# baurst/rbrt

Measured on NVIDIA B200. Metric: Mrays/s, higher is better.
Workload: dtype f32

## Files before the change

rbrt_b200/csrc/api.cu:

```cuda
#include <dlfcn.h>
#include <chrono>
#include <cstdarg>
#include <cstdio>
#include <cstring>
#include "aov.cuh"
#include "bvh_build.cuh"
#include "engine.cuh"
#include "multi.cuh"
#include "query.cuh"
#include "update.cuh"

namespace rbrt {

static thread_local char g_err[512] = "";
void set_error(const char* fmt, ...) {
    va_list ap; va_start(ap, fmt); vsnprintf(g_err, sizeof(g_err), fmt, ap); va_end(ap);
}
int cuda_fail(cudaError_t e, const char* what) {
    set_error("CUDA error %d (%s) at %s", (int)e, cudaGetErrorString(e), what);
    cudaGetLastError();
    return (e == cudaErrorNoDevice || e == cudaErrorInsufficientDriver) ? RBRT_E_NODEVICE : RBRT_E_CUDA;
}
std::recursive_mutex& api_mutex() { static std::recursive_mutex m; return m; }
static uint64_t g_pool_limit = 0;
uint64_t pool_limit_bytes() { return g_pool_limit; }

static int g_device = -1;
static double now_ms() {
    return std::chrono::duration<double, std::milli>(std::chrono::steady_clock::now().time_since_epoch()).count();
}

#define CKA(x) do { cudaError_t e_ = (x); if (e_ != cudaSuccess) return cuda_fail(e_, #x); } while (0)
#define LOCK std::lock_guard<std::recursive_mutex> lock_(api_mutex())

int current_device() { return g_device; }
void set_current_device(int d) { g_device = d; }

static int ensure_device() {
    if (g_device >= 0) { CKA(cudaSetDevice(g_device)); return RBRT_OK; }
    int n = 0;
    cudaError_t e = cudaGetDeviceCount(&n);
    if (e != cudaSuccess || n == 0) {
        set_error("no CUDA device available (%s); rbrt_b200 has no CPU fallback", e != cudaSuccess ? cudaGetErrorString(e) : "device count 0");
        cudaGetLastError();
        return RBRT_E_NODEVICE;
    }
    g_device = 0;
    CKA(cudaSetDevice(0));
    return RBRT_OK;
}

int device_sm_count(int device, int* out) {
    static int cached[64] = {0};
    if (!cached[device & 63]) {
        int smc = 0;
        cudaError_t e = cudaDeviceGetAttribute(&smc, cudaDevAttrMultiProcessorCount, device);
        if (e != cudaSuccess) return cuda_fail(e, "cudaDeviceGetAttribute");
        cached[device & 63] = smc;
    }
    *out = cached[device & 63];
    return RBRT_OK;
// ... 232 lines not shown
        float4* d_tris = (float4*)(base + sc->lay.tris) + 3ull * md.tri_base;
        float4* d_normals = (float4*)(base + sc->lay.nrm) + md.nrm_base;
        float4* d_nodes = (float4*)(base + sc->lay.nodes) + 4ull * md.node_base;
        BuildResult* d_res = (BuildResult*)(base + sc->lay.result) + mi;
        if (mat) {
            Scene::Staging* sg = nullptr;
            { int rc = stage_get(sc, 32, &sg); if (rc) return rc; }
            const float4 m4 = make_float4(mat->albedo.x, mat->albedo.y, mat->albedo.z, mat->param);
            memcpy(sg->p, &m4, 16); memcpy((char*)sg->p + 16, &mat->kind, 4);
            const size_t e = sc->n_elems + mi;
            CKA(cudaMemcpyAsync(base + sc->lay.mat + 16 * e, sg->p, 16, cudaMemcpyHostToDevice, ctx.build));
            CKA(cudaMemcpyAsync(base + sc->lay.kind + 4 * e, (char*)sg->p + 16, 4, cudaMemcpyHostToDevice, ctx.build));
            CKA(cudaEventRecord(sg->done, ctx.build));
        }
        if (flags == RBRT_UPDATE_REBUILD) {
            CKA(build_mesh(ctx, verts, n, n_eff, sc->pad_rel, sc->leaf_size, sc->sah, md, d_mesh, d_tris, d_normals, d_nodes, d_res,
                           on_device ? sc->upd_in : nullptr));
            if (!on_device) {
                { int rc = ensure_event(&sc->t_up1); if (rc) return rc; }
                CKA(build_uploads_done(ctx, sc->t_up1)); uploaded = sc->t_up1;
            }
            { int rc = ensure_event(&sc->rebuild_ev); if (rc) return rc; }
            CKA(cudaMemcpyAsync((BuildResult*)sc->res_h + mi, d_res, sizeof(BuildResult), cudaMemcpyDeviceToHost, ctx.build));
            CKA(cudaEventRecord(sc->rebuild_ev, ctx.build));
            sc->rebuild_pending = true;
        } else {
            const size_t raw_bytes = on_device ? 0 : (36ull * n + 255) & ~255ull;
            char* sbase = nullptr;
            CKA(build_slot_acquire(ctx, raw_bytes + um->scratch_bytes(n_eff), &sbase));
            if (!on_device && n) CKA(cudaMemcpyAsync(sbase, verts, 36ull * n, cudaMemcpyHostToDevice, ctx.copy));
            CKA(build_slot_uploaded(ctx, &uploaded));
            if (on_device) CKA(cudaStreamWaitEvent(ctx.build, sc->upd_in, 0));
            RefitArgs a;
            a.raw = on_device ? verts : (const float*)sbase; a.n_all = n; a.n_eff = n_eff; a.pad_rel = sc->pad_rel;
            a.mesh = d_mesh; a.tris = d_tris; a.normals = d_normals; a.nodes = reinterpret_cast<uint4*>(d_nodes); a.res = d_res;
            CKA((cudaError_t)um->refit(&a, sbase + raw_bytes, ctx.build));
            CKA(build_slot_release(ctx));
            if (on_device) uploaded = nullptr;
        }
    }
    { int rc = update_end(sc, ctx); if (rc) return rc; }
    if (on_device && !receiver) {
        { int rc = ensure_event(&sc->upd_out); if (rc) return rc; }
        CKA(cudaEventRecord(sc->upd_out, ctx.build));
        CKA(cudaStreamWaitEvent(user_st, sc->upd_out, 0));
    }
    if (uploaded) CKA(cudaEventSynchronize(uploaded));
    return RBRT_OK;
}

struct LaunchModule { const char* env; const char* file; const char* what; const char* symbol; void* launch; };
static LaunchModule g_aov_module = {"RBRT_GPU_AOV_LIB", "librbrt_gpu_aov.so", "AOV", "rbrt_aov_launch", nullptr};
static LaunchModule g_query_module = {"RBRT_GPU_QUERY_LIB", "librbrt_gpu_query.so", "query", "rbrt_query_launch", nullptr};
static int load_module(LaunchModule& m) {
    if (!m.launch) {
        std::string path;
        { int rc = module_path(m.env, m.file, &path); if (rc) return rc; }
        void* h = dlopen(path.c_str(), RTLD_NOW | RTLD_LOCAL);
        if (!h) { set_error("the %s module is missing (dlopen %s: %s); build it with make -C rbrt_b200/csrc", m.what, path.c_str(), dlerror()); return RBRT_E_CUDA; }
        void* f = dlsym(h, m.symbol);
        if (!f) { set_error("%s lacks the %s entry point", path.c_str(), m.what); dlclose(h); return RBRT_E_CUDA; }
        m.launch = f;
    }
    return RBRT_OK;
}

struct AovPool { char* buf = nullptr; size_t bytes = 0; unsigned long long* ctr = nullptr; cudaEvent_t e0 = nullptr, e1 = nullptr; };
static AovPool g_aov[64];
static void aov_release_all() {
    int cur = 0; cudaGetDevice(&cur);
    for (int d = 0; d < 64; ++d) {
        AovPool& p = g_aov[d];
        if (!p.buf && !p.ctr && !p.e0) continue;
        cudaSetDevice(d);
        cudaFree(p.buf); cudaFree(p.ctr);
        if (p.e0) cudaEventDestroy(p.e0);
        if (p.e1) cudaEventDestroy(p.e1);
        p = AovPool();
    }
    cudaSetDevice(cur);
}

static int render_aov(const rbrt_scene* scene, const rbrt_camera* cam, uint32_t spp, uint64_t seed, const rbrt_aov_out* out, bool host,
                      cudaStream_t st, rbrt_stats* stats) {
    if (!scene || !cam || !out) { set_error("null argument"); return RBRT_E_INVALID; }
    if (!out->depth && !out->normal && !out->albedo && !out->coverage && !out->hit_kind && !out->elem_idx && !out->tri_idx) {
        set_error("no AOV requested (every member of the output is NULL)"); return RBRT_E_INVALID;
    }
    const uint64_t n = (uint64_t)cam->img_width_pix * cam->img_height_pix;
    if (!n || !spp) { set_error("empty image or zero samples"); return RBRT_E_INVALID; }
    if (n > 0xFFFFFFFFull) { set_error("more than 2^32 - 1 pixels"); return RBRT_E_INVALID; }
    const Scene& sc = *reinterpret_cast<const Scene*>(scene);
    const Replica& rp = sc.rep[0];
    CKA(cudaSetDevice(rp.device));
    const double t0 = now_ms();
    if (stats) memset(stats, 0, sizeof(*stats));
    { int rc = resolve_scene_info(sc, true); if (rc) return rc; }
    { int rc = load_module(g_aov_module); if (rc) return rc; }
    const rbrt_aov_launch_fn launch = reinterpret_cast<rbrt_aov_launch_fn>(g_aov_module.launch);

    AovPool& pool = g_aov[rp.device & 63];
    AovArgs a;
    memset(&a, 0, sizeof(a));
    a.S = rp.dev; a.cam = make_cam(*cam); a.key0 = (uint32_t)seed; a.key1 = (uint32_t)(seed >> 32); a.n_samples = spp;
    a.tiles_x = (cam->img_width_pix + 7) / 8; a.tiles_total = a.tiles_x * ((cam->img_height_pix + 3) / 4);
    a.out = *out;
    if (host) {
        const size_t b1 = a256(4 * n), b3 = a256(12 * n);
        const size_t need = (out->depth ? b1 : 0) + (out->normal ? b3 : 0) + (out->albedo ? b3 : 0) + (out->coverage ? b1 : 0) +
                            (out->hit_kind ? b1 : 0) + (out->elem_idx ? b1 : 0) + (out->tri_idx ? b1 : 0);
        if (pool.bytes < need) {
            cudaFree(pool.buf); pool.buf = nullptr; pool.bytes = 0;
            CKA(cudaMalloc(&pool.buf, need)); pool.bytes = need;
        }
        char* p = pool.buf;
        auto take = [&](const void* want, size_t b) -> char* { if (!want) return nullptr; char* q = p; p += b; return q; };
// ... 609 lines not shown
```

rbrt_b200/csrc/engine.cuh:

```cuda
#pragma once
#include <mutex>
#include <string>
#include <vector>
#include "../../include/rbrt_gpu.h"
#include "common.cuh"

namespace rbrt {

struct IterCtr {
    uint32_t ray_count;
    uint32_t cand_count;
    uint32_t cand_head;
    uint32_t mat_count[3];
    uint32_t shade_head;
    uint32_t pad;
};

enum { ST_RAYS = 0, ST_NAN = 1, ST_NODES = 2, ST_TRIS = 3, ST_CAND = 4, ST_TAIL_NODES = 5, ST_TAIL_TRIS = 6, ST_TAIL_CAND = 7, ST_COUNT = 8 };

struct WaveBuffers {
    uint32_t cap = 0;
    uint32_t depth_cap = 0;
    uint4* rec = nullptr;
    uint32_t* candq = nullptr;
    uint32_t* matq[2][3] = {{nullptr, nullptr, nullptr}, {nullptr, nullptr, nullptr}};
    float4* out = nullptr;
    uint16_t* hist = nullptr;
    IterCtr* ctr = nullptr;
    unsigned long long* stats = nullptr;
    float4* accum = nullptr;
    size_t accum_px = 0;
    uint8_t* rgb = nullptr; float* hdr = nullptr; size_t out_px = 0;
    std::vector<cudaEvent_t> ev;
    size_t bytes = 0;
};

struct ArenaLayout { size_t nodes = 0, tris = 0, nrm = 0, sph = 0, mat = 0, kind = 0, mesh = 0, etris = 0, ekind = 0, result = 0, total = 0; };
struct Replica { int device = 0; char* arena = nullptr; size_t arena_bytes = 0; SceneDev dev{}; int sm_count = 148;
                 cudaEvent_t ready = nullptr; };
struct SceneUse { int device; cudaStream_t stream; cudaEvent_t ev; };

struct Scene {
    int device = 0;
    SceneDev dev{};
    std::vector<MeshDev> meshes_h;
    std::vector<Replica> rep;
    ArenaLayout lay{};
    uint32_t n_elems = 0, n_meshes = 0, n_etris = 0;
    rbrt_scene_info info{};
    int sm_count = 148;
    bool collective = false;
    mutable std::vector<SceneUse> uses;
    void* res_h = nullptr;
    cudaEvent_t info_ev = nullptr, t_up0 = nullptr, t_up1 = nullptr, t_b0 = nullptr, t_b1 = nullptr;
    mutable bool info_resolved = false;
    mutable int build_error = 0;
    double ms_host_create = 0;
    std::vector<uint64_t> mesh_n_all;
    std::vector<uint32_t> elem_kind_h;
    float pad_rel = 0.0f;
    uint32_t leaf_size = 1;
    bool sah = true;
    bool replicated = false;
    cudaEvent_t upd_in = nullptr, upd_out = nullptr;
    cudaEvent_t rebuild_ev = nullptr;
    mutable bool rebuild_pending = false;
    struct Staging { void* p = nullptr; size_t bytes = 0; cudaEvent_t done = nullptr; };
    Staging stage[2];
    int stage_next = 0;
};
int resolve_scene_info(const Scene& sc, bool wait);
void wait_scene_ready(const Scene& sc, int li, cudaStream_t st);
void wait_scene_uses(const Scene& sc, int device, cudaStream_t st);

struct WaveParams {
    SceneDev S;
    CamDev cam[RBRT_MAX_FRAMES];
    ShardDev sh;
    uint32_t key0[RBRT_MAX_FRAMES], key1[RBRT_MAX_FRAMES];
    uint32_t n_frames;
    FastDiv fd_s_count;
// ... 48 lines not shown
```

rbrt_b200/csrc/render.cu:

```cuda
#include <cstdio>
#include <algorithm>
#include <cstdlib>
#include <cstring>
#include "engine.cuh"
#include "intersect.cuh"
#include "cull.cuh"
#include "shade.cuh"

namespace rbrt {

#define FULL_MASK 0xFFFFFFFFu
#define CLS_CAND 3
#define CLS_NONE 7
#define ROUNDS 4

__device__ __forceinline__ uint32_t warp_append(uint32_t* counter, bool pred) {
    uint32_t mask = __ballot_sync(FULL_MASK, pred);
    if (mask == 0) return 0;
    uint32_t lane = threadIdx.x & 31;
    uint32_t leader = __ffs(mask) - 1;
    uint32_t base = 0;
    if (lane == leader) base = atomicAdd(counter, __popc(mask));
    base = __shfl_sync(FULL_MASK, base, leader);
    return base + __popc(mask & ((1u << lane) - 1));
}

__device__ __forceinline__ uint32_t warp_grab(uint32_t* head, uint32_t count) {
    uint32_t base = 0;
    if ((threadIdx.x & 31) == 0) base = atomicAdd(head, count);
    return __shfl_sync(FULL_MASK, base, 0);
}

struct Deferred {
    uint32_t cls;
    uint32_t pid[ROUNDS];
    __device__ __forceinline__ void clear() { cls = 0; for (int r = 0; r < ROUNDS; ++r) { cls |= (uint32_t)CLS_NONE << (3 * r); pid[r] = 0; } }
    __device__ __forceinline__ void set(int r, uint32_t c, uint32_t p) { cls = (cls & ~(7u << (3 * r))) | (c << (3 * r)); pid[r] = p; }
};

__device__ __forceinline__ void flush(const WaveParams& P, uint32_t it, const Deferred& df) {
    IterCtr* c = P.ctr + it;
    const uint32_t lane = threadIdx.x & 31, lt = (1u << lane) - 1;
#pragma unroll
    for (uint32_t k = 0; k < 4; ++k) {
        uint32_t m[ROUNDS], total = 0;
#pragma unroll
        for (int r = 0; r < ROUNDS; ++r) { m[r] = __ballot_sync(FULL_MASK, ((df.cls >> (3 * r)) & 7u) == k); total += __popc(m[r]); }
        if (total == 0) continue;
        uint32_t base = 0;
        if (lane == 0) base = atomicAdd(k == CLS_CAND ? &c->cand_count : &c->mat_count[k], total);
        base = __shfl_sync(FULL_MASK, base, 0);
        uint32_t* q = k == CLS_CAND ? P.candq : P.matq[it & 1][k];
#pragma unroll
        for (int r = 0; r < ROUNDS; ++r) {
            if (m[r] & (1u << lane)) q[base + __popc(m[r] & lt)] = df.pid[r];
            base += __popc(m[r]);
        }
    }
}

// ... 690 lines not shown
            out.elem_idx = elem;
        } else {
            const uint32_t mi = elem - P.S.n_spheres;
            const float4 nn = __ldg(P.S.normals + P.S.meshes[mi].nrm_base + tri); nrm = mk3(nn.x, nn.y, nn.z);
            out.kind = RBRT_HIT_MESH; out.elem_idx = mi; out.tri_idx = tri;
        }
        out.t = t; out.dist = len3(o - p);
        out.point.x = p.x; out.point.y = p.y; out.point.z = p.z;
        out.normal.x = nrm.x; out.normal.y = nrm.y; out.normal.z = nrm.z;
    }
    hits[pid] = out;
}

CamDev make_cam(const rbrt_camera& c) {
    CamDev d;
    d.pos[0] = c.position.x; d.pos[1] = c.position.y; d.pos[2] = c.position.z;
    d.right[0] = c.right.x; d.right[1] = c.right.y; d.right[2] = c.right.z;
    d.up[0] = c.up.x; d.up[1] = c.up.y; d.up[2] = c.up.z;
    d.center[0] = c.img_center_point.x; d.center[1] = c.img_center_point.y; d.center[2] = c.img_center_point.z;
    d.mm_per_pix_hor = c.mm_per_pix_hor; d.mm_per_pix_vert = c.mm_per_pix_vert;
    d.width = c.img_width_pix; d.height = c.img_height_pix;
    return d;
}

static WaveBuffers g_wave[8][64];
WaveBuffers& device_wave_buffers(int device, int pool) { return g_wave[pool & 7][(device >= 0 && device < 64) ? device : 0]; }
struct SplitLane { cudaStream_t aux = nullptr; cudaEvent_t fork = nullptr, acc[2] = {nullptr, nullptr}, join = nullptr; };
static SplitLane g_lane[4][64];
static int ensure_lane(SplitLane& L) {
    if (L.aux) return RBRT_OK;
    cudaError_t e = cudaStreamCreateWithFlags(&L.aux, cudaStreamNonBlocking);
    for (cudaEvent_t* ev : {&L.fork, &L.acc[0], &L.acc[1], &L.join}) if (e == cudaSuccess) e = cudaEventCreateWithFlags(ev, cudaEventDisableTiming);
    if (e != cudaSuccess) return cuda_fail(e, "split lane");
    return RBRT_OK;
}
void release_device_wave_buffers() {
    int cur = 0; cudaGetDevice(&cur);
    for (int p = 0; p < 8; ++p)
        for (int d = 0; d < 64; ++d) if (g_wave[p][d].cap || g_wave[p][d].accum || g_wave[p][d].rgb) { cudaSetDevice(d); free_wave_buffers(g_wave[p][d]); }
    for (int p = 0; p < 4; ++p)
        for (int d = 0; d < 64; ++d) {
            SplitLane& L = g_lane[p][d];
            if (!L.aux) continue;
            cudaSetDevice(d); cudaStreamSynchronize(L.aux); cudaStreamDestroy(L.aux);
            for (cudaEvent_t ev : {L.fork, L.acc[0], L.acc[1], L.join}) if (ev) cudaEventDestroy(ev);
            L = SplitLane();
        }
    cudaSetDevice(cur);
}

void free_wave_buffers(WaveBuffers& wb) {
    cudaFree(wb.rec); cudaFree(wb.candq);
    for (int i = 0; i < 6; ++i) cudaFree(wb.matq[i / 3][i % 3]);
    cudaFree(wb.out); cudaFree(wb.hist); cudaFree(wb.ctr); cudaFree(wb.stats); cudaFree(wb.accum);
    cudaFree(wb.rgb); cudaFree(wb.hdr);
    for (cudaEvent_t e : wb.ev) cudaEventDestroy(e);
    wb = WaveBuffers();
}

#define CKR(x) do { cudaError_t e_ = (x); if (e_ != cudaSuccess) return cuda_fail(e_, #x); } while (0)

static int ensure_wave_buffers(WaveBuffers& wb, uint32_t cap, uint32_t depth) {
    if (wb.cap >= cap && wb.depth_cap >= depth && wb.stats) return RBRT_OK;
    float4* accum = wb.accum; size_t accum_px = wb.accum_px; uint8_t* rgb = wb.rgb; float* hdr = wb.hdr; size_t out_px = wb.out_px;
    std::vector<cudaEvent_t> ev; ev.swap(wb.ev);
    wb.accum = nullptr; wb.rgb = nullptr; wb.hdr = nullptr;
    free_wave_buffers(wb);
    wb.accum = accum; wb.accum_px = accum_px; wb.rgb = rgb; wb.hdr = hdr; wb.out_px = out_px; wb.ev.swap(ev);
    size_t b = 0;
    CKR(cudaMalloc(&wb.rec, 32ull * cap)); b += 32ull * cap;
    CKR(cudaMalloc(&wb.candq, 4ull * cap)); b += 4ull * cap;
    for (int i = 0; i < 6; ++i) { CKR(cudaMalloc(&wb.matq[i / 3][i % 3], 4ull * cap)); b += 4ull * cap; }
    CKR(cudaMalloc(&wb.out, 16ull * cap)); b += 16ull * cap;
    { const uint64_t rows = std::max<uint64_t>(depth, 1); CKR(cudaMalloc(&wb.hist, 2ull * cap * rows)); b += 2ull * cap * rows; }
    CKR(cudaMalloc(&wb.ctr, sizeof(IterCtr) * (depth + 2)));
    CKR(cudaMalloc(&wb.stats, 8 * ST_COUNT));
    wb.cap = cap; wb.depth_cap = depth; wb.bytes = b;
    return RBRT_OK;
}

void note_scene_use(const Scene& sc, int device, cudaStream_t st) {
    static std::mutex mu;
    std::lock_guard<std::mutex> g(mu);
    for (SceneUse& u : sc.uses)
        if (u.device == device && u.stream == st) { cudaEventRecord(u.ev, st); return; }
    SceneUse u{device, st, nullptr};
    if (cudaEventCreateWithFlags(&u.ev, cudaEventDisableTiming) != cudaSuccess) { cudaGetLastError(); return; }
    cudaEventRecord(u.ev, st);
    sc.uses.push_back(u);
}

int make_shard(const rbrt_render_opts& o, uint32_t W, uint32_t H, uint32_t spp, ShardDev* out) {
    ShardDev sh;
    sh.rank = 0; sh.count = 1; sh.s0 = 0; sh.s1 = spp;
    sh.tiles_x = (W + 7) / 8;
    sh.fd_tiles_x = make_fastdiv(sh.tiles_x);
    sh.tiles_total = sh.tiles_x * ((H + 3) / 4);
    if (o.shard_count > 1) {
        if (o.shard_rank >= o.shard_count) { set_error("shard_rank >= shard_count"); return RBRT_E_INVALID; }
        if (o.shard_mode == RBRT_SHARD_TILES) { sh.rank = o.shard_rank; sh.count = o.shard_count; }
        else if (o.shard_mode == RBRT_SHARD_SAMPLES) {
            sh.s0 = (uint32_t)((uint64_t)spp * o.shard_rank / o.shard_count);
            sh.s1 = (uint32_t)((uint64_t)spp * (o.shard_rank + 1) / o.shard_count);
        } else { set_error("shard_count > 1 needs shard_mode TILES or SAMPLES"); return RBRT_E_INVALID; }
    }
    sh.tiles_mine = sh.tiles_total > sh.rank ? (sh.tiles_total - sh.rank + sh.count - 1) / sh.count : 0;
    *out = sh;
    return RBRT_OK;
}

int render_accum(const Scene& sc, int li, const rbrt_camera* cams, const uint64_t* seeds, uint32_t n_frames, uint32_t spp,
                 const rbrt_render_opts* opts, float4* const* d_accum, cudaStream_t st, rbrt_stats* stats, RenderJob* job_out) {
    const Replica& rp = sc.rep[li];
    RenderJob local_job;
    RenderJob& job = job_out ? *job_out : local_job;
    if (!n_frames || n_frames > RBRT_MAX_FRAMES) { set_error("n_frames must be 1..%d", RBRT_MAX_FRAMES); return RBRT_E_INVALID; }
    const rbrt_camera& cam = cams[0];
    const uint32_t W = cam.img_width_pix, H = cam.img_height_pix;
    for (uint32_t f = 1; f < n_frames; ++f)
        if (cams[f].img_width_pix != W || cams[f].img_height_pix != H) { set_error("frames of one batch must have the same image size"); return RBRT_E_INVALID; }
    if (!W || !H || !spp) { set_error("empty image or zero samples"); return RBRT_E_INVALID; }
    if ((uint64_t)W * H > 0x7FFFFFFFull) { set_error("image too large"); return RBRT_E_INVALID; }
    rbrt_render_opts o{}; if (opts) o = *opts;
    const uint32_t max_depth = o.max_depth ? o.max_depth : 50;
    if (max_depth > 1024) { set_error("max_depth > 1024"); return RBRT_E_INVALID; }
    if (o.integrator != 0) { set_error("unknown integrator %u", o.integrator); return RBRT_E_INVALID; }
    ShardDev sh;
    { int rc_sh = make_shard(o, W, H, spp, &sh); if (rc_sh) return rc_sh; }
    const uint32_t P = sh.tiles_mine * 32;
    CKR(cudaEventCreate(&job.ev0)); CKR(cudaEventCreate(&job.ev1));
    const cudaEvent_t ev0 = job.ev0, ev1 = job.ev1;
    wait_scene_ready(sc, li, st);
    for (uint32_t f = 0; f < n_frames; ++f) CKR(cudaMemsetAsync(d_accum[f], 0, 16ull * W * H, st));
    uint32_t launches = 0, iterations = 0, batch_iters = 0;
    const int pool = (int)((o.flags & RBRT_OPT_POOL_MASK) >> RBRT_OPT_POOL_SHIFT);
    const bool split = (o.flags & RBRT_OPT_SPLIT_BATCHES) && !(o.flags & RBRT_OPT_TIME_KERNELS) && sh.s1 - sh.s0 >= 2;
    WaveBuffers* wbs[2] = {&device_wave_buffers(rp.device, pool), split ? &device_wave_buffers(rp.device, 4 + pool) : nullptr};
    WaveBuffers& wb = *wbs[0];
    SplitLane& SL = g_lane[pool][rp.device & 63];
    if (split) { int rc_l = ensure_lane(SL); if (rc_l) return rc_l; }
    cudaStream_t lane_st[2] = {st, split ? SL.aux : st};
    uint32_t lane_iters[2] = {0, 0};
    CKR(cudaEventRecord(ev0, st));
    if (P && sh.s1 > sh.s0) {
        uint32_t target = o.batch_paths;
        const uint64_t PF = (uint64_t)P * n_frames;
        if (PF > 0x7FFFFFFFull) { set_error("batch too large"); return RBRT_E_INVALID; }
        const uint64_t per_path = 76ull + 2ull * std::max<uint64_t>(max_depth, 1);
        const uint64_t limit_paths = pool_limit_bytes() ? std::max<uint64_t>(pool_limit_bytes() / per_path, 1) : ~0ull;
        const uint32_t S_all = sh.s1 - sh.s0, S_half = (S_all + 1) / 2;
        if (!target) {
            const uint64_t want = std::min<uint64_t>(std::min<uint64_t>((uint64_t)(split ? S_half : S_all) * PF, 1ull << 27), limit_paths);
            const uint64_t want_sb = std::max<uint64_t>(want / PF, 1);
            bool have = true;
            for (int l = 0; l < (split ? 2 : 1); ++l) have = have && wbs[l]->cap >= want_sb * PF && wbs[l]->depth_cap >= max_depth;
            if (have) target = (uint32_t)want;
            else {
                size_t free_b = 0, total_b = 0;
                CKR(cudaMemGetInfo(&free_b, &total_b));
                free_b += wb.bytes + (split ? wbs[1]->bytes : 0);
                uint64_t fit = (free_b / 2) / per_path / (split ? 2 : 1);
                target = (uint32_t)(fit < (1ull << 21) ? (1ull << 21) : (fit > (1ull << 27) ? (1ull << 27) : fit));
            }
        }
        if ((uint64_t)target > limit_paths) target = (uint32_t)limit_paths;
        uint64_t S_b64 = (uint64_t)target / PF; if (S_b64 < 1) S_b64 = 1; if (S_b64 > S_all) S_b64 = S_all;
        if (split && S_b64 > S_half) S_b64 = S_half;
        if (S_b64 * PF > 0x7FFFFFFFull) { set_error("batch too large"); return RBRT_E_INVALID; }
        const uint32_t S_b = (uint32_t)S_b64;
        const uint32_t cap = (uint32_t)(S_b64 * PF);
        WaveParams wps[2];
        for (int l = 0; l < (split ? 2 : 1); ++l) {
            WaveBuffers& w = *wbs[l];
            int rc = ensure_wave_buffers(w, cap, max_depth);
            if (rc) return rc;
            WaveParams& wp = wps[l];
            wp.S = rp.dev; wp.sh = sh; wp.n_frames = n_frames;
            for (uint32_t f = 0; f < RBRT_MAX_FRAMES; ++f) {
                const uint32_t g = f < n_frames ? f : 0;
                const uint64_t seed = seeds ? seeds[g] : o.seed;
                wp.cam[f] = make_cam(cams[g]); wp.key0[f] = (uint32_t)seed; wp.key1[f] = (uint32_t)(seed >> 32);
            }
            wp.cap = w.cap; wp.paths_px = P; wp.fd_paths_px = make_fastdiv(P); wp.max_depth = max_depth;
            static const bool no_cull_env = getenv("RBRT_NO_PRIMARY_CULL") != nullptr;
            wp.use_cull = no_cull_env ? 0u : 1u;
            wp.keep_t = 0u;
            const char* thr_env = getenv("RBRT_FETCH_THRESHOLD");
            wp.fetch_thr = thr_env ? (uint32_t)std::min(32, std::max(1, atoi(thr_env))) : FETCH_THRESHOLD;
            const char* tthr_env = getenv("RBRT_TAIL_FETCH_THRESHOLD");
            wp.tail_thr = tthr_env ? (uint32_t)std::min(32, std::max(1, atoi(tthr_env))) : TAIL_FETCH_THRESHOLD;
            wp.rec = w.rec; wp.candq = w.candq;
            for (int i = 0; i < 6; ++i) wp.matq[i / 3][i % 3] = w.matq[i / 3][i % 3];
            wp.out = w.out; wp.hist = w.hist; wp.ctr = w.ctr; wp.stats = w.stats;
        }
        AccumPtrs ap; for (uint32_t f = 0; f < RBRT_MAX_FRAMES; ++f) ap.p[f] = d_accum[f < n_frames ? f : 0];
        if (split) {
            CKR(cudaEventRecord(SL.fork, st));
            CKR(cudaStreamWaitEvent(SL.aux, SL.fork, 0));
        }
        for (int l = 0; l < (split ? 2 : 1); ++l) CKR(cudaMemsetAsync(wbs[l]->stats, 0, 8 * ST_COUNT, lane_st[l]));
        const int sm_count = rp.sm_count;
        const int grid = sm_count * 8;
        int per_sm = 0;
        static int per_sm_cached = 0, fin_per_sm_cached = 0;
        if (!per_sm_cached) CKR(cudaOccupancyMaxActiveBlocksPerMultiprocessor(&per_sm_cached, k_trace<false>, TRACE_THREADS, 0));
        per_sm = per_sm_cached;
        const int grid_trace = sm_count * (per_sm > 0 ? per_sm : 4);
        if (!fin_per_sm_cached) CKR(cudaOccupancyMaxActiveBlocksPerMultiprocessor(&fin_per_sm_cached, k_finish<false, false, false>, 256, 0));
        const int fin_per_sm = fin_per_sm_cached;
        const int grid_fin = sm_count * (fin_per_sm > 0 ? fin_per_sm : 2);
        static int tail_per_sm_cached = 0;
        if (!tail_per_sm_cached) CKR(cudaOccupancyMaxActiveBlocksPerMultiprocessor(&tail_per_sm_cached, k_tail<false, true>, TAIL_THREADS, 0));
        const int grid_tail = sm_count * (tail_per_sm_cached > 0 ? tail_per_sm_cached : 2);
        const char* tail_env = getenv("RBRT_TAIL_RAYS");
        const uint32_t tail_rays = (o.flags & RBRT_OPT_NO_TAIL_KERNEL) ? 0u : (tail_env ? (uint32_t)atoi(tail_env) : (o.trace_mode == RBRT_TRACE_BRUTE ? (uint32_t)grid_fin * 256u : (1u << 18)));
        const bool brute = o.trace_mode == RBRT_TRACE_BRUTE;
        const bool et = rp.dev.n_etris > 0;
        const bool count = (o.flags & RBRT_OPT_COUNT_VISITS) != 0;
        const bool time_kernels = (o.flags & RBRT_OPT_TIME_KERNELS) != 0;
        uint32_t force_it = TAIL_FORCE_IT;
        {
            const char* fenv = getenv("RBRT_TAIL_FORCE_IT");
            uint32_t lg = 0; while (lg < 31 && ((uint64_t)cap >> lg) > (1ull << 18)) ++lg;
            const uint32_t guess = lg + 2 < 2 ? 2 : lg + 2;
            force_it = fenv ? (uint32_t)std::max(1, atoi(fenv)) : std::min<uint32_t>(TAIL_FORCE_IT, guess);
            if (brute) force_it = TAIL_FORCE_IT;
        }
        size_t ev_used = 0;
        auto next_event = [&]() -> cudaEvent_t {
            if (ev_used == wb.ev.size()) { cudaEvent_t e = nullptr; cudaEventCreate(&e); wb.ev.push_back(e); }
            return wb.ev[ev_used++];
        };
        uint32_t batch_no = 0;
        for (uint32_t s_base = sh.s0; s_base < sh.s1; s_base += S_b, ++batch_no) {
            const int l = split ? (int)(batch_no & 1u) : 0;
            WaveParams& wp = wps[l];
            cudaStream_t bs = lane_st[l];
            wp.s_base = s_base; wp.s_count = (sh.s1 - s_base < S_b) ? sh.s1 - s_base : S_b;
            wp.fd_s_count = make_fastdiv(wp.s_count);
            CKR(cudaMemsetAsync(wbs[l]->ctr, 0, sizeof(IterCtr) * (max_depth + 2), bs));
            if (et) k_generate<true><<<grid, 256, 0, bs>>>(wp); else k_generate<false><<<grid, 256, 0, bs>>>(wp);
            ++launches;
            batch_iters = 0;
            const bool no_mesh = sc.info.num_triangles_tested == 0;
            for (uint32_t it = 0; it <= max_depth; ++it) {
                if ((it >= 1 || no_mesh) && tail_rays) {
                    const bool force = it >= force_it || no_mesh;
                    const uint32_t lim = force ? 0xFFFFFFFFu : tail_rays;
                    if (brute) {
                        if (et) { if (count) k_finish<true, true, true><<<grid_fin, 256, 0, bs>>>(wp, it, lim); else k_finish<true, false, true><<<grid_fin, 256, 0, bs>>>(wp, it, lim); }
                        else { if (count) k_finish<true, true, false><<<grid_fin, 256, 0, bs>>>(wp, it, lim); else k_finish<true, false, false><<<grid_fin, 256, 0, bs>>>(wp, it, lim); }
                    } else if (et) { if (count) k_tail<true, true><<<grid_tail, TAIL_THREADS, 0, bs>>>(wp, it, lim); else k_tail<false, true><<<grid_tail, TAIL_THREADS, 0, bs>>>(wp, it, lim); }
                    else { if (count) k_tail<true, false><<<grid_tail, TAIL_THREADS, 0, bs>>>(wp, it, lim); else k_tail<false, false><<<grid_tail, TAIL_THREADS, 0, bs>>>(wp, it, lim); }
                    ++launches;
                    if (force) break;
                }
                if (time_kernels) CKR(cudaEventRecord(next_event(), bs));
                if (brute) { if (count) k_trace_brute<true><<<grid, 256, 0, bs>>>(wp, it); else k_trace_brute<false><<<grid, 256, 0, bs>>>(wp, it); }
                else if (count) k_trace<true><<<grid_trace, TRACE_THREADS, 0, bs>>>(wp, it);
                else k_trace<false><<<grid_trace, TRACE_THREADS, 0, bs>>>(wp, it);
                ++launches; ++iterations; ++batch_iters; ++lane_iters[l];
                if (time_kernels) CKR(cudaEventRecord(next_event(), bs));
                if (it < max_depth) { if (et) k_shade<true><<<grid, 256, 0, bs>>>(wp, it); else k_shade<false><<<grid, 256, 0, bs>>>(wp, it); ++launches; }
            }
            if (split && batch_no > 0) CKR(cudaStreamWaitEvent(bs, SL.acc[l ^ 1], 0));
            k_accumulate<<<dim3((P + 255) / 256, n_frames), 256, 0, bs>>>(wp, ap); ++launches;
            if (split) CKR(cudaEventRecord(SL.acc[l], bs));
            k_sum_rays<<<1, 64, 0, bs>>>(wp); ++launches;
            CKR(cudaGetLastError());
        }
        if (split) {
            CKR(cudaEventRecord(SL.join, SL.aux));
            CKR(cudaStreamWaitEvent(st, SL.join, 0));
        }
    }
    CKR(cudaEventRecord(ev1, st));
    note_scene_use(sc, rp.device, st);
    job.wb = &wb; job.wb2 = split ? wbs[1] : nullptr; job.sh = sh; job.P = P; job.n_frames = n_frames; job.W = W; job.H = H; job.launches = launches; job.iterations = iterations;
    job.batch_iters = batch_iters; job.flags = o.flags; job.max_depth = max_depth; job.rendered = P && sh.s1 > sh.s0;
    if (stats && !job_out) return collect_stats(job, stats);
    return RBRT_OK;
}

int collect_stats(RenderJob& job, rbrt_stats* stats) {
    WaveBuffers& wb = *job.wb;
    const ShardDev& sh = job.sh;
    const uint32_t W = job.W, H = job.H, iterations = job.iterations, max_depth = job.max_depth;
    const cudaEvent_t ev0 = job.ev0, ev1 = job.ev1;
    {
        CKR(cudaEventSynchronize(ev1));
        float ms = 0; CKR(cudaEventElapsedTime(&ms, ev0, ev1));
        unsigned long long h[ST_COUNT] = {0, 0, 0, 0, 0, 0, 0, 0};
        if (wb.stats && job.rendered) CKR(cudaMemcpy(h, wb.stats, sizeof(h), cudaMemcpyDeviceToHost));
        if (job.wb2 && job.wb2->stats && job.rendered) {
            unsigned long long h2[ST_COUNT];
            CKR(cudaMemcpy(h2, job.wb2->stats, sizeof(h2), cudaMemcpyDeviceToHost));
            for (int k = 0; k < ST_COUNT; ++k) h[k] += h2[k];
        }
// ... 21 lines not shown
                float t_first = 0; cudaEventElapsedTime(&t_first, ev0, wb.ev[first]);
                fprintf(stderr, "setup + generate (ev0 -> first trace): %.3f ms; tail kernel ran at it %d\n", t_first, (int)hc[0].pad - 1);
                for (uint32_t it = 0; it < per_batch; ++it) {
                    float t = 0, g = 0; cudaEventElapsedTime(&t, wb.ev[first + 2 * it], wb.ev[first + 2 * it + 1]);
                    if (it + 1 < per_batch) cudaEventElapsedTime(&g, wb.ev[first + 2 * it + 1], wb.ev[first + 2 * it + 2]);
                    else cudaEventElapsedTime(&g, wb.ev[first + 2 * it + 1], ev1);
                    fprintf(stderr, "it %2u rays %9u traversed %9u  lambert %9u metal %9u glass %9u  trace %8.3f ms  then shade+finish %8.3f ms\n", it, hc[it].ray_count,
                            hc[it].cand_count, hc[it].mat_count[0], hc[it].mat_count[1], hc[it].mat_count[2], t, g);
                }
            }
        }
    }
    return RBRT_OK;
}

int finalize(const float4* d_accum, uint32_t W, uint32_t H, uint32_t spp, uint8_t* d_rgb, float* d_hdr, cudaStream_t st) {
    size_t n = (size_t)W * H;
    if (!n || !spp) { set_error("empty image or zero samples"); return RBRT_E_INVALID; }
    float inv = 1.0f / (float)spp;
    k_finalize<<<(unsigned)((n + 255) / 256), 256, 0, st>>>(d_accum, n, inv, d_rgb, d_hdr);
    CKR(cudaGetLastError());
    return RBRT_OK;
}

int trace_rays_device(const Scene& sc, const rbrt_ray* d_rays, uint64_t n, uint32_t mode, rbrt_hit* d_hits,
                      unsigned long long* d_stats, cudaStream_t st) {
    if (!n) return RBRT_OK;
    wait_scene_ready(sc, 0, st);
    unsigned g = (unsigned)((n + 255) / 256);
    if (mode == RBRT_TRACE_BRUTE) k_trace_rays<true><<<g, 256, 0, st>>>(sc.dev, d_rays, n, d_hits, d_stats);
    else k_trace_rays<false><<<g, 256, 0, st>>>(sc.dev, d_rays, n, d_hits, d_stats);
    CKR(cudaGetLastError());
    return RBRT_OK;
}

int scatter_device(const rbrt_scatter_in* d_in, uint64_t n, uint64_t seed, rbrt_scatter_out* d_out, cudaStream_t st) {
    if (!n) return RBRT_OK;
    k_scatter_kat<<<(unsigned)((n + 255) / 256), 256, 0, st>>>(d_in, n, (uint32_t)seed, (uint32_t)(seed >> 32), d_out);
    CKR(cudaGetLastError());
    return RBRT_OK;
}

int trace_rays_wavefront(const Scene& sc, const rbrt_ray* d_rays, uint64_t n, rbrt_hit* d_hits, unsigned long long* d_stats, cudaStream_t st) {
    const Replica& rp = sc.rep[0];
    WaveBuffers& wb = device_wave_buffers(rp.device, 0);
    wait_scene_ready(sc, 0, st);
    const uint64_t chunk = 1ull << 24;
    static int per_sm_cached = 0;
    if (!per_sm_cached) CKR(cudaOccupancyMaxActiveBlocksPerMultiprocessor(&per_sm_cached, k_trace<false>, TRACE_THREADS, 0));
    const bool et = rp.dev.n_etris > 0;
    for (uint64_t base = 0; base < n; base += chunk) {
        const uint32_t m = (uint32_t)std::min<uint64_t>(chunk, n - base);
        const uint32_t cap = (m + 31u) & ~31u;
        int rc = ensure_wave_buffers(wb, std::max<uint32_t>(cap, 1u << 16), 50);
        if (rc) return rc;
        WaveParams wp;
        memset(&wp, 0, sizeof(wp));
        wp.S = rp.dev; wp.n_frames = 1; wp.cap = wb.cap; wp.paths_px = cap; wp.fd_paths_px = make_fastdiv(cap); wp.fd_s_count = make_fastdiv(1);
        wp.s_count = 1; wp.max_depth = 50; wp.fetch_thr = FETCH_THRESHOLD; wp.tail_thr = TAIL_FETCH_THRESHOLD; wp.keep_t = 1u;
        wp.rec = wb.rec; wp.candq = wb.candq;
        for (int i = 0; i < 6; ++i) wp.matq[i / 3][i % 3] = wb.matq[i / 3][i % 3];
        wp.out = wb.out; wp.hist = wb.hist; wp.ctr = wb.ctr; wp.stats = wb.stats;
        CKR(cudaMemsetAsync(wb.ctr, 0, sizeof(IterCtr) * 52, st));
        CKR(cudaMemsetAsync(wb.stats, 0, 8 * ST_COUNT, st));
        CKR(cudaMemsetAsync(wb.out, 0xFF, 16ull * cap, st));
        const int grid = rp.sm_count * 8;
        if (et) k_rays_stage_a<true><<<grid, 256, 0, st>>>(wp, d_rays + base, m); else k_rays_stage_a<false><<<grid, 256, 0, st>>>(wp, d_rays + base, m);
        if (d_stats) k_trace<true><<<rp.sm_count * std::max(per_sm_cached, 1), TRACE_THREADS, 0, st>>>(wp, 0);
        else k_trace<false><<<rp.sm_count * std::max(per_sm_cached, 1), TRACE_THREADS, 0, st>>>(wp, 0);
        k_rays_collect<<<(m + 255) / 256, 256, 0, st>>>(wp, d_rays + base, m, d_hits + base);
        CKR(cudaGetLastError());
        if (d_stats) {
            CKR(cudaStreamSynchronize(st));
            unsigned long long h[ST_COUNT], acc[ST_COUNT];
            CKR(cudaMemcpy(h, wb.stats, sizeof(h), cudaMemcpyDeviceToHost));
            CKR(cudaMemcpy(acc, d_stats, sizeof(acc), cudaMemcpyDeviceToHost));
            for (int k = 0; k < ST_COUNT; ++k) acc[k] += h[k];
            CKR(cudaMemcpy(d_stats, acc, sizeof(acc), cudaMemcpyHostToDevice));
        }
    }
    note_scene_use(sc, rp.device, st);
    return RBRT_OK;
}

int primary_rays_device(const rbrt_camera& cam, uint64_t seed, uint32_t sample, rbrt_ray* d_rays, cudaStream_t st) {
    size_t n = (size_t)cam.img_width_pix * cam.img_height_pix;
    if (!n) return RBRT_OK;
    k_primary_rays<<<(unsigned)((n + 255) / 256), 256, 0, st>>>(make_cam(cam), (uint32_t)seed, (uint32_t)(seed >> 32), sample, d_rays);
    CKR(cudaGetLastError());
    return RBRT_OK;
}

}
```

Before: 7798.

## Reorder candidate ray queue by path id before each trace iteration

Adds a separately loaded order module that, each bounce, marks surviving path ids in a bitmap, counts bits per block, then rewrites the candidate queue in sorted path-id order. The intent is to restore memory coherence of per-path record accesses in the trace and shade kernels after compaction scrambles the queue. It runs only when the queue count is at least about four million rays and the pad flag is zero, and adds three extra kernel launches per iteration plus bitmap memory. It also makes rendering depend on a dlopen'ed library being present.

```diff
diff --git a/rbrt_b200/csrc/api.cu b/rbrt_b200/csrc/api.cu
--- a/rbrt_b200/csrc/api.cu
+++ b/rbrt_b200/csrc/api.cu
@@ -7,6 +7,7 @@
 #include "bvh_build.cuh"
 #include "engine.cuh"
 #include "multi.cuh"
+#include "order.cuh"
 #include "query.cuh"
 #include "update.cuh"
 
@@ -345,6 +346,7 @@
 struct LaunchModule { const char* env; const char* file; const char* what; const char* symbol; void* launch; };
 static LaunchModule g_aov_module = {"RBRT_GPU_AOV_LIB", "librbrt_gpu_aov.so", "AOV", "rbrt_aov_launch", nullptr};
 static LaunchModule g_query_module = {"RBRT_GPU_QUERY_LIB", "librbrt_gpu_query.so", "query", "rbrt_query_launch", nullptr};
+static LaunchModule g_order_module = {"RBRT_GPU_ORDER_LIB", "librbrt_gpu_order.so", "queue-order", "rbrt_order_launch", nullptr};
 static int load_module(LaunchModule& m) {
     if (!m.launch) {
         std::string path;
@@ -355,6 +357,14 @@
         if (!f) { set_error("%s lacks the %s entry point", path.c_str(), m.what); dlclose(h); return RBRT_E_CUDA; }
         m.launch = f;
     }
+    return RBRT_OK;
+}
+
+int order_module(rbrt_order_launch_fn* out) {
+    static std::mutex mu;
+    std::lock_guard<std::mutex> g(mu);
+    { int rc = load_module(g_order_module); if (rc) return rc; }
+    *out = reinterpret_cast<rbrt_order_launch_fn>(g_order_module.launch);
     return RBRT_OK;
 }
 
diff --git a/rbrt_b200/csrc/engine.cuh b/rbrt_b200/csrc/engine.cuh
--- a/rbrt_b200/csrc/engine.cuh
+++ b/rbrt_b200/csrc/engine.cuh
@@ -27,6 +27,7 @@
     float4* out = nullptr;
     uint16_t* hist = nullptr;
     IterCtr* ctr = nullptr;
+    uint32_t* order = nullptr;
     unsigned long long* stats = nullptr;
     float4* accum = nullptr;
     size_t accum_px = 0;
diff --git a/rbrt_b200/csrc/order.cu b/rbrt_b200/csrc/order.cu
--- /dev/null
+++ b/rbrt_b200/csrc/order.cu
@@ -0,0 +1,112 @@
+#include "order.cuh"
+
+namespace rbrt {
+namespace {
+
+#define ORD_FULL 0xFFFFFFFFu
+#define ORD_THREADS 256
+#define ORD_WARPS (ORD_THREADS / 32)
+#define ORD_ROUNDS 8
+#define ORD_WORDS_PER_BLOCK (ORD_WARPS * ORD_ROUNDS * 32)
+#define ORD_MARK_BLOCKS 2048
+static_assert(ORD_WORDS_PER_BLOCK * 32 == ORDER_PIDS_PER_BLOCK, "order.cuh states the block size");
+
+__device__ __forceinline__ bool nothing_to_do(const uint32_t* count, uint32_t min_count, const uint32_t* pad) {
+    const uint32_t n = *count;
+    return n == 0u || n < min_count || *pad != 0u;
+}
+
+__device__ __forceinline__ uint32_t block_total(uint32_t v, uint32_t* s_red) {
+    for (int off = 16; off; off >>= 1) v += __shfl_xor_sync(ORD_FULL, v, off);
+    if ((threadIdx.x & 31) == 0) s_red[threadIdx.x >> 5] = v;
+    __syncthreads();
+    uint32_t t = 0;
+#pragma unroll
+    for (int w = 0; w < ORD_WARPS; ++w) t += s_red[w];
+    __syncthreads();
+    return t;
+}
+
+__global__ void __launch_bounds__(ORD_THREADS) k_order_mark(const uint32_t* __restrict__ queue, const uint32_t* count, uint32_t min_count, const uint32_t* pad,
+                                                            uint32_t* __restrict__ bitmap) {
+    if (nothing_to_do(count, min_count, pad)) return;
+    const uint32_t n = *count;
+    const uint32_t n_all = (n + 31u) & ~31u;
+    for (uint32_t i = blockIdx.x * ORD_THREADS + threadIdx.x; i < n_all; i += gridDim.x * ORD_THREADS) {
+        const bool have = i < n;
+        const uint32_t pid = have ? queue[i] : 0xFFFFFFFFu;
+        const uint32_t word = pid >> 5;
+        const uint32_t peers = __match_any_sync(ORD_FULL, word);
+        const uint32_t bits = __reduce_or_sync(peers, have ? 1u << (pid & 31u) : 0u);
+        if (have && (threadIdx.x & 31u) == (uint32_t)(__ffs(peers) - 1)) atomicOr(bitmap + word, bits);
+    }
+}
+
+__global__ void __launch_bounds__(ORD_THREADS) k_order_count(const uint32_t* __restrict__ bitmap, uint32_t n_words, const uint32_t* count,
+                                                             uint32_t min_count, const uint32_t* pad, uint32_t* __restrict__ block_sums) {
+    if (nothing_to_do(count, min_count, pad)) return;
+    __shared__ uint32_t s_red[ORD_WARPS];
+    const uint32_t w0 = blockIdx.x * ORD_WORDS_PER_BLOCK;
+    uint32_t c = 0;
+    for (uint32_t k = threadIdx.x; k < ORD_WORDS_PER_BLOCK; k += ORD_THREADS)
+        if (w0 + k < n_words) c += __popc(bitmap[w0 + k]);
+    c = block_total(c, s_red);
+    if (threadIdx.x == 0) block_sums[blockIdx.x] = c;
+}
+
+__global__ void __launch_bounds__(ORD_THREADS) k_order_emit(uint32_t* __restrict__ queue, uint32_t* __restrict__ bitmap, uint32_t n_words,
+                                                            const uint32_t* count, uint32_t min_count, const uint32_t* pad,
+                                                            const uint32_t* __restrict__ block_sums) {
+    if (nothing_to_do(count, min_count, pad)) return;
+    __shared__ uint32_t s_pid[ORD_WARPS][32 * 32];
+    __shared__ uint32_t s_red[ORD_WARPS], s_warp[ORD_WARPS];
+    const uint32_t lane = threadIdx.x & 31, warp = threadIdx.x >> 5;
+    uint32_t before = 0;
+    for (uint32_t b = threadIdx.x; b < blockIdx.x; b += ORD_THREADS) before += block_sums[b];
+    before = block_total(before, s_red);
+    const uint32_t wbase = blockIdx.x * ORD_WORDS_PER_BLOCK + warp * ORD_ROUNDS * 32;
+    uint32_t bits[ORD_ROUNDS], mine = 0;
+#pragma unroll
+    for (int r = 0; r < ORD_ROUNDS; ++r) {
+        const uint32_t w = wbase + 32u * r + lane;
+        bits[r] = w < n_words ? bitmap[w] : 0u;
+        if (bits[r]) bitmap[w] = 0u;
+        mine += __popc(bits[r]);
+    }
+    for (int off = 16; off; off >>= 1) mine += __shfl_xor_sync(ORD_FULL, mine, off);
+    if (lane == 0) s_warp[warp] = mine;
+    __syncthreads();
+    uint32_t out = before;
+    for (uint32_t w = 0; w < warp; ++w) out += s_warp[w];
+    uint32_t* const stage = s_pid[warp];
+#pragma unroll
+    for (int r = 0; r < ORD_ROUNDS; ++r) {
+        const uint32_t c = __popc(bits[r]);
+        uint32_t incl = c;
+        for (int off = 1; off < 32; off <<= 1) { const uint32_t y = __shfl_up_sync(ORD_FULL, incl, off); if (lane >= (uint32_t)off) incl += y; }
+        const uint32_t round_total = __shfl_sync(ORD_FULL, incl, 31);
+        if (round_total == 0u) continue;
+        uint32_t x = bits[r], k = incl - c;
+        const uint32_t pid0 = (wbase + 32u * r + lane) << 5;
+        while (x) { stage[k++] = pid0 + (uint32_t)(__ffs(x) - 1); x &= x - 1u; }
+        __syncwarp();
+        for (uint32_t i = lane; i < round_total; i += 32) queue[out + i] = stage[i];
+        __syncwarp();
+        out += round_total;
+    }
+}
+
+}
+}
+
+extern "C" int rbrt_order_launch(uint32_t* queue, const uint32_t* count, uint32_t min_count, const uint32_t* pad, uint32_t* bitmap,
+                                 uint32_t* block_sums, uint32_t n_paths, cudaStream_t stream) {
+    if (!n_paths) return (int)cudaSuccess;
+    const uint32_t n_words = (n_paths + 31u) / 32u;
+    const uint32_t blocks = (n_words + ORD_WORDS_PER_BLOCK - 1) / ORD_WORDS_PER_BLOCK;
+    const uint32_t mark_blocks = (n_paths + ORD_THREADS - 1) / ORD_THREADS < ORD_MARK_BLOCKS ? (n_paths + ORD_THREADS - 1) / ORD_THREADS : ORD_MARK_BLOCKS;
+    rbrt::k_order_mark<<<mark_blocks, ORD_THREADS, 0, stream>>>(queue, count, min_count, pad, bitmap);
+    rbrt::k_order_count<<<blocks, ORD_THREADS, 0, stream>>>(bitmap, n_words, count, min_count, pad, block_sums);
+    rbrt::k_order_emit<<<blocks, ORD_THREADS, 0, stream>>>(queue, bitmap, n_words, count, min_count, pad, block_sums);
+    return (int)cudaGetLastError();
+}
diff --git a/rbrt_b200/csrc/order.cuh b/rbrt_b200/csrc/order.cuh
--- /dev/null
+++ b/rbrt_b200/csrc/order.cuh
@@ -0,0 +1,16 @@
+#pragma once
+#include <cstdint>
+#include <cuda_runtime.h>
+
+#define ORDER_PIDS_PER_BLOCK 65536u
+
+extern "C" {
+typedef int (*rbrt_order_launch_fn)(uint32_t* queue, const uint32_t* count, uint32_t min_count, const uint32_t* pad, uint32_t* bitmap,
+                                    uint32_t* block_sums, uint32_t n_paths, cudaStream_t stream);
+
+#define ORDER_MIN_RAYS (1u << 22)
+}
+
+namespace rbrt {
+int order_module(rbrt_order_launch_fn* out);
+}
diff --git a/rbrt_b200/csrc/render.cu b/rbrt_b200/csrc/render.cu
--- a/rbrt_b200/csrc/render.cu
+++ b/rbrt_b200/csrc/render.cu
@@ -6,6 +6,7 @@
 #include "intersect.cuh"
 #include "cull.cuh"
 #include "shade.cuh"
+#include "order.cuh"
 
 namespace rbrt {
 
@@ -802,7 +803,7 @@
 void free_wave_buffers(WaveBuffers& wb) {
     cudaFree(wb.rec); cudaFree(wb.candq);
     for (int i = 0; i < 6; ++i) cudaFree(wb.matq[i / 3][i % 3]);
-    cudaFree(wb.out); cudaFree(wb.hist); cudaFree(wb.ctr); cudaFree(wb.stats); cudaFree(wb.accum);
+    cudaFree(wb.out); cudaFree(wb.hist); cudaFree(wb.ctr); cudaFree(wb.order); cudaFree(wb.stats); cudaFree(wb.accum);
     cudaFree(wb.rgb); cudaFree(wb.hdr);
     for (cudaEvent_t e : wb.ev) cudaEventDestroy(e);
     wb = WaveBuffers();
@@ -810,7 +811,7 @@
 
 #define CKR(x) do { cudaError_t e_ = (x); if (e_ != cudaSuccess) return cuda_fail(e_, #x); } while (0)
 
-static int ensure_wave_buffers(WaveBuffers& wb, uint32_t cap, uint32_t depth) {
+static int ensure_wave_buffers(WaveBuffers& wb, uint32_t cap, uint32_t depth, cudaStream_t st) {
     if (wb.cap >= cap && wb.depth_cap >= depth && wb.stats) return RBRT_OK;
     float4* accum = wb.accum; size_t accum_px = wb.accum_px; uint8_t* rgb = wb.rgb; float* hdr = wb.hdr; size_t out_px = wb.out_px;
     std::vector<cudaEvent_t> ev; ev.swap(wb.ev);
@@ -824,6 +825,11 @@
     CKR(cudaMalloc(&wb.out, 16ull * cap)); b += 16ull * cap;
     { const uint64_t rows = std::max<uint64_t>(depth, 1); CKR(cudaMalloc(&wb.hist, 2ull * cap * rows)); b += 2ull * cap * rows; }
     CKR(cudaMalloc(&wb.ctr, sizeof(IterCtr) * (depth + 2)));
+    {
+        const size_t words = (cap + 31ull) / 32 + (cap + ORDER_PIDS_PER_BLOCK - 1ull) / ORDER_PIDS_PER_BLOCK;
+        CKR(cudaMalloc(&wb.order, 4 * words)); b += 4 * words;
+        CKR(cudaMemsetAsync(wb.order, 0, 4 * words, st));
+    }
     CKR(cudaMalloc(&wb.stats, 8 * ST_COUNT));
     wb.cap = cap; wb.depth_cap = depth; wb.bytes = b;
     return RBRT_OK;
@@ -919,10 +925,12 @@
         if (S_b64 * PF > 0x7FFFFFFFull) { set_error("batch too large"); return RBRT_E_INVALID; }
         const uint32_t S_b = (uint32_t)S_b64;
         const uint32_t cap = (uint32_t)(S_b64 * PF);
+        rbrt_order_launch_fn order_launch = nullptr;
+        { int rc = order_module(&order_launch); if (rc) return rc; }
         WaveParams wps[2];
         for (int l = 0; l < (split ? 2 : 1); ++l) {
             WaveBuffers& w = *wbs[l];
-            int rc = ensure_wave_buffers(w, cap, max_depth);
+            int rc = ensure_wave_buffers(w, cap, max_depth, lane_st[l]);
             if (rc) return rc;
             WaveParams& wp = wps[l];
             wp.S = rp.dev; wp.sh = sh; wp.n_frames = n_frames;
@@ -988,12 +996,18 @@
             cudaStream_t bs = lane_st[l];
             wp.s_base = s_base; wp.s_count = (sh.s1 - s_base < S_b) ? sh.s1 - s_base : S_b;
             wp.fd_s_count = make_fastdiv(wp.s_count);
+            WaveBuffers& w = *wbs[l];
+            const uint32_t n_paths = n_frames * wp.s_count * P;
+            auto order = [&](uint32_t* queue, const uint32_t* count) {
+                return (cudaError_t)order_launch(queue, count, ORDER_MIN_RAYS, &w.ctr[0].pad, w.order, w.order + (w.cap + 31ull) / 32, n_paths, bs);
+            };
             CKR(cudaMemsetAsync(wbs[l]->ctr, 0, sizeof(IterCtr) * (max_depth + 2), bs));
             if (et) k_generate<true><<<grid, 256, 0, bs>>>(wp); else k_generate<false><<<grid, 256, 0, bs>>>(wp);
             ++launches;
             batch_iters = 0;
             const bool no_mesh = sc.info.num_triangles_tested == 0;
             for (uint32_t it = 0; it <= max_depth; ++it) {
+                if (it >= 1 && !brute) CKR(order(w.candq, &w.ctr[it].cand_count));
                 if ((it >= 1 || no_mesh) && tail_rays) {
                     const bool force = it >= force_it || no_mesh;
                     const uint32_t lim = force ? 0xFFFFFFFFu : tail_rays;
@@ -1121,7 +1135,7 @@
     for (uint64_t base = 0; base < n; base += chunk) {
         const uint32_t m = (uint32_t)std::min<uint64_t>(chunk, n - base);
         const uint32_t cap = (m + 31u) & ~31u;
-        int rc = ensure_wave_buffers(wb, std::max<uint32_t>(cap, 1u << 16), 50);
+        int rc = ensure_wave_buffers(wb, std::max<uint32_t>(cap, 1u << 16), 50, st);
         if (rc) return rc;
         WaveParams wp;
         memset(&wp, 0, sizeof(wp));
```

Result: slower. 7658, median of 6 (-1.8%).
